# zahmedy/PyTorch-Distributed-Data-Parallel-DDP-Trainer

Measured on AMD Instinct MI355X. Metric: images/sec MNIST SimpleCNN DDP at 1/2/4/8 MI355X; DDP scaling efficiency, higher is better.
Workload: dtype bf16; 1 GPU; model=SimpleCNN (520,586 params), global_batch=32, per_rank_batch=32, image=1x28x28, parallelism=dp1, engine=fused hipGraph, graph_steps=7, graph_head=0, fuse_level=3, level3=True, params_finite=True, bucket_allreduce=none, params_identical_across_ranks=True, ranks_seen=1, force_allreduce=False, inlaunch_allreduce=False

## Files before the change

### csrc/bindings.cpp

```cpp
#include <torch/extension.h>
#include <c10/hip/HIPStream.h>

#include <optional>

#include "kernels/launchers.h"
#include "runtime/runtime.h"

namespace py = pybind11;
using at::Tensor;
using namespace ddp_amd;

extern "C" const char ddp_amd_source_hash_str[];

namespace {

hipStream_t cur_stream() { return c10::hip::getCurrentHIPStream().stream(); }

void check_cuda(const Tensor& t, const char* name) {
  TORCH_CHECK(t.is_cuda(), name, " must be a GPU tensor");
  TORCH_CHECK(t.is_contiguous(), name, " must be contiguous");
}
void check(const Tensor& t, const char* name, at::ScalarType st) {
  check_cuda(t, name);
  TORCH_CHECK(t.scalar_type() == st, name, " has dtype ", t.scalar_type(), ", expected ", st);
// ... 987 lines not shown
               b.a1 = bf(need("a1", at::kBFloat16, B * HW * c.C1));
               b.a2 = bf(need("a2", at::kBFloat16, B * HW * c.C2));
               b.dz2 = bf(need("dz2", at::kBFloat16, B * HW * c.C2));
               b.dz1 = bf(need("dz1", at::kBFloat16, B * HW * c.C1));
             }
             b.fc_part = need("fc_part", at::kFloat, 2L * conv3x3_dgrad_blocks(B, c.H, c.W, c.pxt_fwd) * c.NO).data_ptr<float>();
             b.dlogits = need("dlogits", at::kFloat, B * c.NO).data_ptr<float>();
             b.loss_rows = need("loss_rows", at::kFloat, B).data_ptr<float>();
             b.loss_hist = need("loss_hist", at::kFloat, 1).data_ptr<float>();
             b.w2slab = need("w2slab", at::kFloat, (long)conv3x3_wgrad_blocks(B, c.H, c.wgrad_rows) * (9L * c.C1 * c.C2 + c.C2)).data_ptr<float>();
             b.w1slab = need("w1slab", at::kFloat, (long)conv3x3_dgrad_blocks(B, c.H, c.W, c.pxt_dgrad) * 320).data_ptr<float>();
             b.step_ctr = need("step_ctr", at::kInt, 1).data_ptr<int>();
             b.xb = need("xb", at::kByte, B * HW).data_ptr<unsigned char>();
             b.yb = need("yb", at::kInt, B).data_ptr<int>();
             if (t.contains("sync_flags")) {
               long nfl = L3_IMG_OFF;
               if (c.fuse_level >= 3) nfl = std::max(nfl, (long)L3_IMG_OFF + (long)FWD_DZ_CNT_STRIDE * (B + 2));
               b.sync_flags = need("sync_flags", at::kInt, nfl).data_ptr<int>();
               b.sync_err = need("sync_err", at::kInt, 1).data_ptr<int>();
             }
             Tensor images = need("images", at::kByte, HW);
             b.images = images.data_ptr<unsigned char>();
             Tensor labels = need("labels", at::kInt, 1);
             b.labels = labels.data_ptr<int>();
             Tensor idx = need("idx", at::kInt, 1);
             b.idx = idx.data_ptr<int>();
             b.n_idx = (int)idx.numel();
             b.n_rows = (int)std::min<long>(images.numel() / HW, labels.numel());
             if (cfgd.contains("epoch_order") && cfgd["epoch_order"].cast<bool>()) b.idx = nullptr;
             TORCH_CHECK(conv3x3_wgrad_lds(c.W, c.C1, c.C2, c.wgrad_rows, true, es) <= 160 * 1024, "wgrad rows too large");
             return std::make_shared<SimpleCNNEngine>(c, b, comm, buckets);
           }),
// ... 26 lines not shown
```

### csrc/kernels/common.h

```cpp
#pragma once
#include <hip/hip_runtime.h>
#include <stdint.h>

#include "kernels/types.h"

namespace ddp_amd {

typedef __attribute__((ext_vector_type(8))) short bf16x8;
typedef __attribute__((ext_vector_type(4))) short bf16x4;
typedef __attribute__((ext_vector_type(4))) float f32x4;
typedef __attribute__((address_space(3))) bf16x4 lds_bf16x4;
typedef __attribute__((address_space(3))) char lds_char;
__device__ __forceinline__ lds_bf16x4* lds_ptr4(lds_char* base, int elem_off) {
  return (lds_bf16x4*)(base + 2 * elem_off);
}
typedef __attribute__((ext_vector_type(2))) __bf16 bf16x2v;

constexpr int WAVE = 64;

__device__ __forceinline__ void lds_barrier() {
  asm volatile("s_waitcnt lgkmcnt(0)\n\ts_barrier" ::: "memory");
}

namespace {
// ... 242 lines not shown
__device__ __forceinline__ float lane_bcast(float v, int lane) {
  return __builtin_bit_cast(float, __builtin_amdgcn_readlane(__builtin_bit_cast(int, v), lane));
}
__device__ __forceinline__ float wave_sum(float v) {
  v = row16_sum(v);
  return (lane_bcast(v, 0) + lane_bcast(v, 16)) + (lane_bcast(v, 32) + lane_bcast(v, 48));
}
__device__ __forceinline__ float sum16(float v) { return row16_sum(v); }
__device__ __forceinline__ float wave_max(float v) {
  v = row16_max(v);
  return fmaxf(fmaxf(lane_bcast(v, 0), lane_bcast(v, 16)), fmaxf(lane_bcast(v, 32), lane_bcast(v, 48)));
}

constexpr int XENT_MAX_BLK = 16;
constexpr int XENT_PRE_Q = 4;
template <typename Ld>
__device__ __forceinline__ float xent_logit_acc(int b, int o, int HW, int CH, int NO, Ld ld) {
  const int p0 = b * HW;
  const int kb0 = p0 / CH, kb1 = (p0 + HW - 1) / CH;
  const int slot0 = kb0 * CH == p0 ? 0 : 1;
  float a = 0.f;
#pragma unroll
  for (int j = 0; j < XENT_MAX_BLK; ++j) {
    const int kb = min(kb0 + j, kb1);
    const float v = ld((kb * 2 + (j == 0 ? slot0 : 0)) * NO + o);
    a += (kb0 + j <= kb1) ? v : 0.f;
  }
  return a;
}
__device__ __forceinline__ float xent_row_dl(const float* x, int NO, int o, int label, float gscale,
                                             float* loss) {
  label = label < 0 ? 0 : (label >= NO ? NO - 1 : label);
  float mx = x[0];
  for (int k = 1; k < NO; ++k) mx = fmaxf(mx, x[k]);
  float se = 0.f;
  for (int k = 0; k < NO; ++k) se += __expf(x[k] - mx);
  const float inv = 1.f / se;
  if (o == 0 && loss) *loss = mx + __logf(se) - x[label];
  return (__expf(x[o] - mx) * inv - (o == label ? 1.f : 0.f)) * gscale;
}
struct XentPre {
  int lab0;
  float bias_o;
// ... 78 lines not shown
```

### csrc/kernels/conv3x3.hip

```cpp
#include <algorithm>
#include <stdexcept>

#include <cstdio>
#include <cstdlib>

#include "kernels/conv3x3_fwd.h"

namespace ddp_amd {

size_t conv3x3_fwd_lds(int W, int Cin, int pxt, bool a1x, int es) {
  return fwd_stage_lds(W, Cin, pxt, a1x, es) + fc_epi_lds(pxt, FC_MAX_NOF);
}

size_t conv3x3_dgrad_lds(int W, int Cout, int pxt, bool fuse_w1, int es) {
  const size_t XR = 64 * pxt + 2 * W + 2;
  const int pad = es == 2 ? 16 : 8;
  return (size_t)es * ((size_t)32 * (9 * Cout + pad) + XR * (Cout + pad)) +
         (fuse_w1 ? sizeof(float) * (XR + 4 * 320) + 4 * 64 * pxt : 0);
}

bool conv3x3_fwd_dz_fits(int B, int H, int W, int pxt, int es) {
  return es == 4 ? fwd_dz_fits<float>(B, H, W, pxt) : fwd_dz_fits<bf16_t>(B, H, W, pxt);
}

// ... 29 lines not shown
bool conv3x3_step_head_fits(int nx, int B) {
  if (B <= 0 || nx <= 0) return false;
  const long nf = ((long)B * 28 * 28 + 63) / 64;
  const bool ok = (long)conv3x3_step_head_slots() >= nx + nf;
  if (!ok && std::getenv("DDP_AMD_XAR_DEBUG"))
    fprintf(stderr, "[ddp_amd] step head does not fit: %d resident slots < %ld blocks\n", conv3x3_step_head_slots(),
            nx + nf);
  return ok;
}

bool conv3x3_step_head(const BwdXar& x, int* done_fc, int* done_conv, const bf16_t* Wt, const float* bias,
                       bf16_t* Y, int B, const bf16_t* wfc, float* fc_part, const C1Src& c1, const FwdDz& dz,
                       int* err, hipStream_t s, const ShadowSet* late) {
  const int nx = x.nblk0 + x.nblk1;
  const char* bad = !x.args ? "all-reduce arguments" : x.nblk0 < 0 || x.nblk1 <= 0 ? "the conv bucket's blocks"
                   : !done_fc || !done_conv ? "bucket-done counters" : !dz.dz2 || !dz.img_cnt || !dz.fc_bias
                   ? "the level-3 forward's dZ2 outputs" : !wfc ? "the fc weight shadow" : !c1.x ? "the images" : nullptr;
  if (bad) throw std::runtime_error(std::string("conv3x3_step_head: missing ") + bad);
  if (!conv3x3_step_head_fits(nx, B)) return false;
  const long nf = ((long)B * 28 * 28 + 63) / 64;
  const size_t lds = std::max(conv3x3_fwd_lds(28, 32, 1, true, 2), (size_t)64 + sizeof(XgmiArgs));
  FwdMerge mg;
  mg.args = x.args;
  mg.nblk0 = x.nblk0;
  mg.nblk1 = x.nblk1;
  mg.fc_done = done_fc;
  mg.conv_done = done_conv;
  mg.err = err;
  if (late) mg.late = *late;
  auto k = step_head_kernel<bf16_t>;
  lds_optin(k, lds);
// ... 4 lines not shown
template <typename T>
static void fwd_launch(const T* X, const T* Wt, const float* bias, T* Y, int B, int H, int W, int Cin,
                       int Cout, bool relu, const T* wfc, float* fc_part, int pxt, hipStream_t s,
                       const C1Src* c1, const FwdDz* dz) {
  const long P = (long)B * H * W;
  const int per_blk = 64 * pxt;
  const dim3 grid((unsigned)((P + per_blk - 1) / per_blk), Cout / 64);
  const bool a1x = c1 != nullptr;
  const size_t lds = conv3x3_fwd_lds(W, Cin, pxt, a1x, (int)sizeof(T));
  const bool fc = wfc != nullptr;
  const C1Src cs = a1x ? *c1 : C1Src();
  const bool g = simplecnn_geom(H, W, Cin, Cout);
  const FwdDz dzo = dz ? *dz : FwdDz();
  if (dz) {
    if (!g || !fc || !a1x || !(pxt == 1 || pxt == 2) || !(sizeof(T) == 2 ? (void*)dz->dz2 : (void*)dz->dz2_f32) ||
        !dz->img_cnt || !dz->fc_bias)
      throw std::runtime_error("conv3x3_fwd: the level-3 dZ2 epilogue is the SimpleCNN forward with the fc "
                               "epilogue and the conv1 recompute");
    if constexpr (sizeof(T) == 2) {
      if (pxt == 2 && fwd_dz_occ2(grid.x)) {
        auto k = fwd_dz_kernel<T, 2, 2>();
        lds_optin(k, lds);
        hipLaunchKernelGGL(k, grid, dim3(512), lds, s, X, Wt, bias, Y, B, H, W, Cin, Cout, wfc, fc_part, cs, dzo);
        return;
      }
    }
    auto k = pxt == 2 ? fwd_dz_kernel<T, 2>() : fwd_dz_kernel<T, 1>();
    lds_optin(k, lds);
    hipLaunchKernelGGL(k, grid, dim3(256 * pxt), lds, s, X, Wt, bias, Y, B, H, W, Cin, Cout, wfc, fc_part, cs, dzo);
    return;
  }
// ... 143 lines not shown
```

### csrc/kernels/conv3x3_fwd.h

```cpp
#pragma once

#include "kernels/conv3x3_body.h"

namespace ddp_amd {

constexpr unsigned long long FWD_DZ_WAIT_TICKS = 2000000;
#ifndef DDP_AMD_F32_FC_PREFETCH
#define DDP_AMD_F32_FC_PREFETCH 0
#endif
constexpr bool F32_FC_PREFETCH = DDP_AMD_F32_FC_PREFETCH;
#ifndef DDP_AMD_FWD_PF_SPLIT
#define DDP_AMD_FWD_PF_SPLIT 1
#endif

struct FwdMerge {
  const XgmiArgs* args = nullptr;
  int nblk0 = 0, nblk1 = 0;
  int* fc_done = nullptr;
  int* conv_done = nullptr;
  int* err = nullptr;
  ShadowSet late{};
};
constexpr int MRG_ERR = 5;

// ... 117 lines not shown
```

### csrc/kernels/conv3x3_fwd_body.inc.h

```cpp
  using P = Prec<T>;
  constexpr bool F32 = sizeof(T) == 4;
  static_assert(!DZ || (NOF == 10 && A1X), "level-3 dZ2 needs the fc epilogue and the conv1 recompute");
  static_assert(!MRG || (DZ && !F32), "the merged forward is the bf16 level-3 forward");
  constexpr int CE = P::CE;
  DDP_STAMP(STAMP_K_CONV_FWD, 0);
  DDP_GEOM_OVERRIDE();
  constexpr int CH = 16 * NW * PXT, NT = NW * 64;
  const int lane = threadIdx.x & 63, wave = threadIdx.x >> 6;
  const int HW = H * W;
  const long Ptot = (long)B * HW;
  const int co0 = by * 64;
  const int KW = 9 * Cin, WS = KW + P::PAD, XS = Cin + P::PAD;
  const int XR = CH + 2 * W + 2;
  T* sW = reinterpret_cast<T*>(smem);
  T* sX = sW + 64 * WS;
  const long P0 = (long)bx * CH;
  const long Pbase = P0 - W - 1;

  const int wc = KW / CE;
  const int xc = Cin / CE;
  if (A1X && c1.zero_i32)
    for (int i = threadIdx.x; i < c1.zero_per_block; i += NT) {
      const long z = (long)bx * c1.zero_per_block + i;
      if (z < c1.zero_total) c1.zero_i32[z] = 0;
    }
  Conv1Group cg;
  if constexpr (!MRG) {
  if (A1X) cg = conv1_group_load(c1.w, c1.b, wave & 3);
  stage2<(64 / NW) * (F32 ? 2 : 1), NT>(64 * wc,
             [&](int i) { const int r = i / wc, c = (i - r * wc) * CE; return ld16(Wt + (long)(co0 + r) * KW + c); },
             [&](int i, bf16x8 v) { const int r = i / wc, c = (i - r * wc) * CE; st16(sW + r * WS + c, v); },
             A1X ? 0 : XR * xc,
             [&](int i) {
               const int r = i / xc, c = (i - r * xc) * CE;
               const long Pq = Pbase + r;
               return (Pq >= 0 && Pq < Ptot) ? ld16(X + Pq * Cin + c) : zero8();
             },
             [&](int i, bf16x8 v) { const int r = i / xc, c = (i - r * xc) * CE; st16(sX + r * XS + c, v); });
  }
  if (A1X) {
    float* sxx = reinterpret_cast<float*>(sX + XR * XS);
    const int NXX = XR + 2 * W + 2;
    const int base = c1.bi.base();
    for (int r = threadIdx.x; r < NXX; r += NT) {
      const long Pq = Pbase - W - 1 + r;
      float v = 0.f;
      if (Pq >= 0 && Pq < Ptot) {
        const int n = (int)(Pq / HW), rm = (int)(Pq - (long)n * HW);
        const int row = c1.bi.row(n, base);
        const unsigned char u = c1.x[(long)row * HW + rm];
        v = (float)u / 255.0f;
        if (c1.xb_out && Pq >= P0 && Pq < P0 + CH) {
          c1.xb_out[Pq] = u;
          if (rm == 0) c1.yb_out[n] = c1.labels[row];
        }
      }
      sxx[r] = v;
    }
// ... 217 lines not shown
    lds_barrier();
    if ((int)threadIdx.x < 2 * NOF) {
      const int slot = threadIdx.x / NOF, o = threadIdx.x - (threadIdx.x / NOF) * NOF;
      const long img = P0 / HW + slot;
      float acc_o = 0.f;
#pragma unroll
      for (int tile = 0; tile < NW * PXT; ++tile) {
        const long tp = P0 + tile * 16;
        const bool in = tp < Ptot && tp / HW == img;
#pragma unroll
        for (int g = 0; g < 4; ++g) {
          const float v = s_fc[(tile * 4 + g) * NOF + o];
          acc_o += in ? v : 0.f;
        }
      }
      float* dst = fc_part + ((long)bx * 2 + slot) * NOF + o;
      if constexpr (DZ || NOA2) st_wt(dst, acc_o);
      else *dst = acc_o;
    }
  }
  DDP_STAMP(STAMP_K_CONV_FWD, 4);
  if constexpr (DZ) {
    const int HWi = H * W;
    const int img0 = (int)(P0 / HWi);
    const long plast = (P0 + CH < Ptot ? P0 + CH : Ptot) - 1;
    const int nimg = (int)(plast / HWi) - img0 + 1;
    float* s_lg = s_fc + NW * PXT * 4 * NOF;
    float* s_dl = s_lg + 2 * NOF;
    auto store_a2 = [&]() {
#pragma unroll
      for (int pt = 0; pt < PXT; ++pt)
#pragma unroll
        for (int t = 0; t < 4; ++t) {
          const int co = co0 + 16 * t + 4 * (lane >> 4);
          if (!valid[pt]) continue;
          if constexpr (F32) st_wt(reinterpret_cast<float4*>(Y + Pp[pt] * Cout + co), a2q[pt][t]);
          else st_wt(reinterpret_cast<uint2*>(Y + Pp[pt] * Cout + co), a2pk[pt][t]);
        }
    };
    DDP_STAMP(STAMP_K_FWD_DZ, 0);
    if (wave != 0) store_a2();
    if (wave == 0) {
      int label = 0;
      if (lane < 2 * NOF) {
        const int im = img0 + (lane >= NOF ? 1 : 0);
        if (im < B) label = c1.labels[c1.bi.row(im, c1.bi.base())];
      }
      asm volatile("s_waitcnt vmcnt(0)" ::: "memory");
      DDP_STAMP(STAMP_K_FWD_DZ, 1);
      if (lane < nimg)
        __hip_atomic_fetch_add(dzo.img_cnt + (img0 + lane) * FWD_DZ_CNT_STRIDE, 1, __ATOMIC_RELAXED,
                               __HIP_MEMORY_SCOPE_AGENT);
      store_a2();
      {
        const int im = img0 + (lane < nimg ? lane : 0);
        const int kb0 = im * HWi / CH, kb1 = (im * HWi + HWi - 1) / CH;
        const int want = kb1 - kb0 + 1;
        const unsigned long long t0 = __builtin_amdgcn_s_memrealtime();
        while (true) {
          const int v = lane < nimg ? __hip_atomic_load(dzo.img_cnt + im * FWD_DZ_CNT_STRIDE, __ATOMIC_RELAXED,
                                                        __HIP_MEMORY_SCOPE_AGENT)
                                    : want;
          if (__all(v >= want)) break;
          if (__builtin_amdgcn_s_memrealtime() - t0 > FWD_DZ_WAIT_TICKS) {
            if (lane == 0 && dzo.err) __hip_atomic_store(dzo.err, 3, __ATOMIC_RELAXED, __HIP_MEMORY_SCOPE_AGENT);
            break;
          }
          __builtin_amdgcn_s_sleep(1);
        }
      }
      DDP_STAMP(STAMP_K_FWD_DZ, 2);
      if (lane < 2 * NOF) {
        const int slot = lane >= NOF ? 1 : 0, o = lane - slot * NOF;
        if (slot < nimg) {
          const float a = xent_logit_acc(img0 + slot, o, HWi, CH, NOF, [&](int i) {
            return __hip_atomic_load(fc_part + i, __ATOMIC_RELAXED, __HIP_MEMORY_SCOPE_AGENT);
          });
          s_lg[lane] = (MRG ? __hip_atomic_load(dzo.fc_bias + o, __ATOMIC_RELAXED, __HIP_MEMORY_SCOPE_AGENT)
                            : dzo.fc_bias[o]) + a;
        }
      }
      DDP_STAMP(STAMP_K_FWD_DZ, 4);
      asm volatile("s_waitcnt lgkmcnt(0)" ::: "memory");
      if (lane < 2 * NOF) {
        const int slot = lane >= NOF ? 1 : 0, o = lane - slot * NOF;
        if (slot < nimg) {
          float lossv = 0.f;
          const float d = xent_row_dl(s_lg + slot * NOF, NOF, o, label, dzo.gscale, &lossv);
          s_dl[lane] = d;
          if (dzo.dl_out && (slot == 1 || P0 == (long)img0 * HWi)) {
            const int im = img0 + slot;
            dzo.dl_out[im * NOF + o] = d;
            if (o == 0) dzo.loss_rows[im] = lossv;
          }
        }
      }
    }
    lds_barrier();
    DDP_STAMP(STAMP_K_FWD_DZ, 3);
#pragma unroll
    for (int pt = 0; pt < PXT; ++pt) {
      const long tp = P0 + (wave * PXT + pt) * 16;
      const float* dl = s_dl + (tp / HWi != img0 ? NOF : 0);
      float d[NOF];
#pragma unroll
      for (int o = 0; o < NOF; ++o) d[o] = dl[o];
#pragma unroll
      for (int t = 0; t < 4; ++t) {
        if constexpr (!PFW && !F32) __builtin_amdgcn_sched_barrier(0);
// ... 35 lines not shown
```

### csrc/kernels/fc_bwd_body.h

```cpp
#pragma once
#include "kernels/common.h"
#include "kernels/launchers.h"

namespace ddp_amd {

constexpr int FCB_RB = 8;

template <int CPL>
struct ColF {
  float v[CPL];
};
template <int CPL>
__device__ __forceinline__ ColF<CPL> ldc(const bf16_t* p) {
  ColF<CPL> r;
  if constexpr (CPL == 2) {
    const unsigned u = *reinterpret_cast<const unsigned*>(p);
    r.v[0] = __builtin_bit_cast(float, u << 16);
    r.v[1] = __builtin_bit_cast(float, u & 0xffff0000u);
  } else {
    const uint2 u = *reinterpret_cast<const uint2*>(p);
    r.v[0] = __builtin_bit_cast(float, u.x << 16);
    r.v[1] = __builtin_bit_cast(float, u.x & 0xffff0000u);
    r.v[2] = __builtin_bit_cast(float, u.y << 16);
    r.v[3] = __builtin_bit_cast(float, u.y & 0xffff0000u);
// ... 57 lines not shown
  if ((XENT || ex.loss_rows) && ex.loss_out) {
    const float* lr = XENT ? s_loss : ex.loss_rows;
    const int at = ex.step_ctr ? *ex.step_ctr : 0;
    float acc = 0.f;
    for (int b0 = 0; b0 < B; b0 += 64) {
      const float v = b0 + lane < B ? lr[b0 + lane] : 0.f;
      const int nb = B - b0 < 64 ? B - b0 : 64;
      for (int k = 0; k < nb; ++k)
        acc += __builtin_bit_cast(float, __builtin_amdgcn_readlane(__builtin_bit_cast(int, v), k));
    }
    if (lane == 63) {
      ex.loss_out[at] = acc / (float)B;
      if (last && ex.step_inc) *ex.step_inc = at + 1;
    }
  }
  if (ex.zero_i32 && (last || !ex.last_ctr))
    for (int i = lane; i < ex.n_zero; i += 64) ex.zero_i32[(long)i * ex.zero_stride] = 0;
}

constexpr int FCDW_LD = 12;
template <int MAXB, typename T>
__device__ __forceinline__ void fc_dw_wave_chunk(const float* s_dl, const T* __restrict__ X,
                                                 float* __restrict__ dW, float scale, int B, long K,
                                                 const FcBwdExtras& ex, long col0) {
  constexpr bool F32 = sizeof(T) == 4;
  constexpr int NO = 10, VW = 8, RPV = (MAXB + VW - 1) / VW;
  const int lane = threadIdx.x & 63;
  const long col = col0 + 2 * lane;
  const bool active = col < K;
  const long cc = active ? col : 0;
  typedef __attribute__((ext_vector_type(2))) int i32x2_t;
  const int vo4 = (int)cc * 4, vo2 = (int)cc * 2;
// ... 263 lines not shown
```

### csrc/kernels/launchers.h

```cpp
#pragma once
#include <hip/hip_runtime.h>
#include <stdint.h>

#include "kernels/types.h"

namespace ddp_amd {

void stamps_set(void* buf);

void conv1_fwd(const void* x, bool x_is_u8, BatchIdx bi, const float* w, const float* b, bf16_t* y,
               int B, int H, int W, int Cout, hipStream_t s);
void conv1_fwd(const void* x, bool x_is_u8, BatchIdx bi, const float* w, const float* b, float* y,
               int B, int H, int W, int Cout, hipStream_t s);
int conv1_wgrad_blocks(int B, int H, int W, int chunk);
void conv1_wgrad(const void* x, bool x_is_u8, BatchIdx bi, const bf16_t* dy, const bf16_t* yact,
                 float* slab, int B, int H, int W, int Cout, int chunk, hipStream_t s);
void conv1_wgrad(const void* x, bool x_is_u8, BatchIdx bi, const float* dy, const float* yact,
                 float* slab, int B, int H, int W, int Cout, int chunk, hipStream_t s);

constexpr int FWD_DZ_CNT_STRIDE = 64;
struct FwdDz {
  bf16_t* dz2 = nullptr;
  float* dz2_f32 = nullptr;
  int* img_cnt = nullptr;
  const float* fc_bias = nullptr;
  float gscale = 1.f;
  int* err = nullptr;
  float* dl_out = nullptr;
  float* loss_rows = nullptr;
};
bool conv3x3_fwd_dz_fits(int B, int H, int W, int pxt, int es = 2);
void conv3x3_fwd(const bf16_t* X, const bf16_t* Wt, const float* bias, bf16_t* Y, int B, int H,
                 int W, int Cin, int Cout, bool relu, const bf16_t* wfc, float* fc_part, int NO,
                 int pxt, hipStream_t s, const C1Src* c1 = nullptr, const FwdDz* dz = nullptr);
void conv3x3_fwd(const float* X, const float* Wt, const float* bias, float* Y, int B, int H,
                 int W, int Cin, int Cout, bool relu, const float* wfc, float* fc_part, int NO,
                 int pxt, hipStream_t s, const C1Src* c1 = nullptr, const FwdDz* dz = nullptr);
void conv3x3_dgrad(const bf16_t* dY, const bf16_t* Yact, const bf16_t* WT, const bf16_t* Xact,
                   bf16_t* dX, int B, int H, int W, int Cin, int Cout, const void* x0, bool x0_u8,
// ... 130 lines not shown
  const int* labels32 = nullptr;
  BatchIdx bi{};
  float gscale = 1.f;
  SgdArgs sgd{};
  float* p_w = nullptr;
  float* m_w = nullptr;
  bf16_t* sh_plain = nullptr;
  bf16_t* sh_frag = nullptr;
  float* sh_frag32 = nullptr;
  int frag_HW = 0, frag_C = 0;
  int sys_store = 0;
  int* last_ctr = nullptr;
  float* p_b = nullptr;
  float* m_b = nullptr;
  int* step_inc = nullptr;
  int* zero_i32 = nullptr;
  int n_zero = 0, zero_stride = 1;
  int last_n = 0;
};
struct BwdFc {
  const void* a2 = nullptr;
  const float* dl = nullptr;
  float* dW = nullptr;
  float scale = 1.f;
  long K = 0;
  int nconv = 0, fc0 = 0, nfc = 0;
  FcBwdExtras ex{};
};
size_t fc_bwd_lds(int B, int NO, bool xent, long npart = 0);
void noop(int blocks, int* sink, hipStream_t s);
// ... 109 lines not shown
```

### csrc/runtime/engine.cpp

```cpp
#include <algorithm>
#include <cstdio>
#include <cstdlib>
#include <cstring>

#include "runtime/runtime.h"

namespace ddp_amd {

SimpleCNNEngine::SimpleCNNEngine(const EngineConfig& cfg, const EngineBuffers& buf,
                                 std::shared_ptr<Comm> comm, std::vector<EngineBucket> buckets)
    : cfg_(cfg), b_(buf), comm_(std::move(comm)), buckets_(std::move(buckets)) {
  if (cfg_.C1 != 32) throw std::runtime_error("engine: fused conv1 wgrad needs C1 == 32");
  if (cfg_.C2 % 64 != 0) throw std::runtime_error("engine: C2 must be a multiple of 64");
  if ((cfg_.H * cfg_.W) % 16 != 0) throw std::runtime_error("engine: H*W must be a multiple of 16");
  if (cfg_.NO != 10) throw std::runtime_error("engine: the fused fc epilogue is built for 10 classes");
  if (cfg_.f32 && (cfg_.fuse_level < 1 || cfg_.store_a1 != 0))
    throw std::runtime_error("engine: fp32 mode needs fuse_level >= 1 (level 1 or 3) and store_a1 0");
  if (cfg_.f32 && !(b_.a2_f32 && b_.dz2_f32 && b_.w2t_f32 && b_.wfc_frag32))
    throw std::runtime_error("engine: fp32 mode needs the a2 / dz2 / w2t / wfc_frag32 fp32 buffers");
  const long conv0 = std::min(std::min(b_.off_w2, b_.off_b2), std::min(b_.off_w1, b_.off_b1));
  const long fc_hi = std::max(b_.off_wfc + (long)cfg_.NO * cfg_.H * cfg_.W * cfg_.C2, b_.off_bfc + cfg_.NO);
  if (fc_hi > conv0) throw std::runtime_error("engine: fc gradients must precede the conv gradients");
  long prev_end = 0;
  for (const EngineBucket& bk : buckets_) {
// ... 6 lines not shown
  for (int s : stage_) stage_used_[s] = true;
  xch_.assign(buckets_.size(), -1);
  DDP_HIP_CHECK(hipStreamCreateWithFlags(&cs_, hipStreamNonBlocking));
  DDP_HIP_CHECK(hipStreamCreateWithFlags(&ms_, hipStreamNonBlocking));
  for (hipEvent_t* e : {&e_b0_, &e_b1_, &e_d0_, &e_d1_, &e_fwd_, &e_fc_})
    DDP_HIP_CHECK(hipEventCreateWithFlags(e, hipEventDisableTiming));
  l3_fits_.assign(cfg_.max_batch + 1, -1);
  if (b_.sync_err) {
    DDP_HIP_CHECK(hipHostMalloc(reinterpret_cast<void**>(&err_host_), sizeof(int),
                                hipHostMallocCoherent | hipHostMallocMapped));
    *err_host_ = 0;
    int* dev = nullptr;
    DDP_HIP_CHECK(hipHostGetDevicePointer(reinterpret_cast<void**>(&dev), err_host_, 0));
    b_.sync_err = dev;
  }
}

SimpleCNNEngine::~SimpleCNNEngine() {
  if (process_exiting()) return;
  if (cs_) hipStreamSynchronize(cs_);
  destroy_graph();
  for (hipEvent_t e : {e_b0_, e_b1_, e_d0_, e_d1_, e_fwd_, e_fc_}) hipEventDestroy(e);
  for (XarArgs& e : xar_cache_) hipFree(const_cast<XgmiArgs*>(e.dev));
  if (err_host_) hipHostFree(err_host_);
}

void SimpleCNNEngine::destroy_graph() {
  if (graph_exec_) hipGraphExecDestroy(graph_exec_);
  if (graph_) hipGraphDestroy(graph_);
  graph_exec_ = nullptr;
  graph_ = nullptr;
  graph_steps_ = 0;
}

void SimpleCNNEngine::synchronize() {
  DDP_HIP_CHECK(hipStreamSynchronize(cs_));
  if (const int e = sync_error()) {
    throw std::runtime_error(std::string("engine: an in-launch hand-off wait timed out (") +
                             (e == 2 ? "fused slab reduction" : e == XAR_ERR ? "in-launch all-reduce"
// ... 79 lines not shown
  const bool pair_mode = dist && use_x && f1 && cfg_.dist_mode >= 3 && sync_ok_for_xar();
  if (fred || l3 || pair_mode) {
    const int nfwd = conv3x3_dgrad_blocks(B, H, W, cfg_.pxt_fwd);
    const int nsync = SYNC_RED_INTS + ((l3 || pair_mode) ? L3_FC_INTS : 0);
    c1.zero_i32 = b_.sync_flags;
    c1.zero_per_block = (nsync + nfwd - 1) / nfwd;
    c1.zero_total = nsync;
  }
  if (!l3 && plain_stale_) {
    refresh_shadows();
    plain_stale_ = false;
  }
  FwdDz dzo;
  if (l3) {
    dzo.dz2 = b_.dz2;
    dzo.img_cnt = b_.sync_flags + L3_IMG_OFF;
    dzo.fc_bias = P + b_.off_bfc;
    dzo.gscale = 1.f / (float)B;
    dzo.err = b_.sync_err;
    dzo.dl_out = b_.dlogits;
    dzo.loss_rows = b_.loss_rows;
  }
  const bool xar_mode = dist && use_x && l3 &&
                        ((cfg_.dist_mode == 2 && xar_plan_ok_) || cfg_.dist_mode >= 3);
  const bool one_stream = xar_mode || pair_mode;
  const bool fc_role = l3 && (!dist || xar_mode) && cfg_.l3_fc_role &&
                       conv3x3_bwd_fc_role_ok(H, W, C1, C2, cfg_.pxt_dgrad, cfg_.wgrad_split);
  const bool ov = dist && use_x && l3 && fc_role && cfg_.dist_mode == 4;
  if ((parts & (PART_HEAD | PART_AR)) && !ov && parts != PART_ALL)
    throw std::runtime_error("engine: a split step needs the dist_mode 4 chain");
  const C1Src* pc1 = f1 ? &c1 : nullptr;
// ... 14 lines not shown
  sh_all.count = l3 ? 3 : 4;
  const SgdArgs sa{cfg_.lr, cfg_.momentum, cfg_.dampening, cfg_.weight_decay, cfg_.nesterov,
                   cfg_.maximize, first_momentum_step ? 1 : 0, 1};
  float* M = b_.momentum;
  bool head_used = false;
  if (parts & PART_HEAD) {
    if (first_momentum_step) throw std::runtime_error("engine: the step head runs the steady-state SGD only");
    ShadowSet sh_head = sh_all, late{};
    if (late_shadow_ok(b_.off_w2, n_w2s)) {
      sh_head.r[1] = sh_all.r[2];
      sh_head.count = 2;
      late.r[0] = sh_all.r[1];
      late.count = 1;
    }
    BwdXar hx;
    int* mc = b_.sync_flags + L3_IMG_OFF + (long)FWD_DZ_CNT_STRIDE * cfg_.max_batch;
    if (cfg_.pxt_fwd == 1 && B == cfg_.max_batch) {
      if (!make_xar(hx, sa, M, sh_head)) throw std::runtime_error("engine: the step head needs the pair plan");
      hx.step_ctr = nullptr;
      head_used = conv3x3_step_head(hx, mc, mc + FWD_DZ_CNT_STRIDE, b_.w2_bf16, P + b_.off_b2, b_.a2, B,
                                    b_.wfc_frag, b_.fc_part, c1, dzo, b_.sync_err, cs_, &late);
    }
    if (!head_used) {
      if (!make_xar(hx, sa, M, sh_all)) throw std::runtime_error("engine: the step head needs the pair plan");
      hx.step_ctr = nullptr;
      xgmi_allreduce_pair(hx, cs_);
    }
    DDP_HIP_CHECK(hipGetLastError());
  }
  if ((parts & PART_FWD) || ((parts & PART_HEAD) && !head_used)) {
    if (!f1) conv1_fwd(b_.images, true, bi, P + b_.off_w1, P + b_.off_b1, b_.a1, B, H, W, C1, cs_);
// ... 27 lines not shown
  ex.sys_store = use_x ? 1 : 0;
  if (fopt) {
    ex.sgd = sa;
    ex.p_w = P + b_.off_wfc;
    ex.m_w = M ? M + b_.off_wfc : nullptr;
    ex.sh_plain = b_.wfc_bf16;
    ex.sh_frag = b_.wfc_frag;
    ex.frag_HW = HW;
    ex.frag_C = C2;
  }
  BwdFc fcr;
  std::function<void(hipStream_t)> fc_launch;
  if (l3) {
    ex.part = nullptr;
    ex.loss_rows = b_.loss_rows;
    ex.zero_i32 = dzo.img_cnt;
    ex.n_zero = ov ? cfg_.max_batch + 2 : B;
    ex.zero_stride = FWD_DZ_CNT_STRIDE;
    if (fc_role) {
      if (fopt) {
        ex.p_b = P + b_.off_bfc;
        ex.m_b = M ? M + b_.off_bfc : nullptr;
        ex.step_inc = b_.step_ctr;
      }
      if (ov) ex.step_inc = b_.step_ctr;
      ex.sh_plain = nullptr;
      fcr.a2 = b_.a2;
      fcr.dl = b_.dlogits;
      fcr.dW = fopt ? nullptr : G + b_.off_wfc;
      fcr.scale = inv_ws;
      fcr.K = (long)HW * C2;
      fcr.ex = ex;
    } else {
// ... 246 lines not shown
  const bool pair_mode = dist && use_x && cfg_.dist_mode >= 3 && sync_ok_for_xar();
  if (fred || l3 || pair_mode) {
    const int nfwd = conv3x3_dgrad_blocks(B, H, W, cfg_.pxt_fwd);
    const int nsync = SYNC_RED_INTS + ((l3 || pair_mode) ? L3_FC_INTS : 0);
    c1.zero_i32 = b_.sync_flags;
    c1.zero_per_block = (nsync + nfwd - 1) / nfwd;
    c1.zero_total = nsync;
  }
  const long n_w2 = (long)C2 * 9 * C1, w2row = n_w2 + C2, n_fc = (long)NO * HW * C2;
  const SgdArgs sa{cfg_.lr, cfg_.momentum, cfg_.dampening, cfg_.weight_decay, cfg_.nesterov,
                   cfg_.maximize, first_momentum_step ? 1 : 0, 1};
  const bool fopt = !dist && cfg_.fuse_opt;
  FwdDz dzo;
  if (l3) {
    dzo.dz2_f32 = b_.dz2_f32;
    dzo.img_cnt = b_.sync_flags + L3_IMG_OFF;
    dzo.fc_bias = P + b_.off_bfc;
    dzo.gscale = 1.f / (float)B;
    dzo.err = b_.sync_err;
    dzo.dl_out = b_.dlogits;
    dzo.loss_rows = b_.loss_rows;
  }
  const bool xar_mode = dist && use_x && l3 &&
                        ((cfg_.dist_mode == 2 && xar_plan_ok_) || cfg_.dist_mode >= 3);
  const bool one_stream = xar_mode || pair_mode;
  const bool fc_role = l3 && (!dist || xar_mode) && cfg_.l3_fc_role &&
                       conv3x3_bwd_fc_role_ok(H, W, C1, C2, cfg_.pxt_dgrad, cfg_.wgrad_split);

  conv3x3_fwd(static_cast<const float*>(nullptr), P + b_.off_w2, P + b_.off_b2, b_.a2_f32, B, H, W, C1, C2,
              true, b_.wfc_frag32, b_.fc_part, NO, cfg_.pxt_fwd, cs_, &c1, l3 ? &dzo : nullptr);
  FcBwdExtras ex;
  ex.dbias = G + b_.off_bfc;
  ex.dbias_scale = inv_ws;
  ex.loss_out = b_.loss_hist;
  ex.step_ctr = b_.step_ctr;
  ex.sys_store = use_x ? 1 : 0;
  if (l3) {
    ex.loss_rows = b_.loss_rows;
    ex.zero_i32 = dzo.img_cnt;
    ex.n_zero = B;
    ex.zero_stride = FWD_DZ_CNT_STRIDE;
  } else {
    ex.part = b_.fc_part;
    ex.HW = HW;
    ex.CH = 64 * cfg_.pxt_fwd;
    ex.fc_bias = P + b_.off_bfc;
    ex.labels32 = b_.yb;
    ex.bi = bid;
    ex.gscale = 1.f / (float)B;
  }
  if (fopt) {
    ex.sgd = sa;
    ex.p_w = P + b_.off_wfc;
    ex.m_w = M ? M + b_.off_wfc : nullptr;
    ex.sh_frag32 = b_.wfc_frag32;
    ex.frag_HW = HW;
// ... 176 lines not shown
```

### csrc/runtime/runtime.h

```cpp
#pragma once
#include <hip/hip_runtime.h>
#include <rccl/rccl.h>

#include <functional>
#include <memory>
#include <stdexcept>
#include <string>
#include <vector>

#include "kernels/launchers.h"
#include "runtime/bucket_state.h"

#define DDP_HIP_CHECK(expr)                                                              \
  do {                                                                                   \
    hipError_t _e = (expr);                                                              \
    if (_e != hipSuccess)                                                                \
      throw std::runtime_error(std::string("HIP error ") + hipGetErrorString(_e) + " at " + \
                               __FILE__ + ":" + std::to_string(__LINE__) + ": " #expr);  \
  } while (0)

#define DDP_NCCL_CHECK(expr)                                                             \
  do {                                                                                   \
    ncclResult_t _r = (expr);                                                            \
    if (_r != ncclSuccess)                                                               \
// ... 125 lines not shown
  float* wfc_frag32 = nullptr;
  bf16_t *a1, *a2, *dz2, *dz1;
  float *fc_part, *dlogits, *loss_rows, *loss_hist, *w2slab, *w1slab;
  int* step_ctr;
  unsigned char* xb;
  int* yb;
  int* sync_flags = nullptr;
  int* sync_err = nullptr;
  const unsigned char* images;
  const int* labels;
  const int* idx;
  int n_idx, n_rows;
};

constexpr int L3_FC_INTS = 32;
constexpr int L3_IMG_OFF = SYNC_RED_INTS + L3_FC_INTS;

struct EngineConfig {
  int max_batch, H, W, C1, C2, NO;
  int pxt_fwd, pxt_dgrad, wgrad_rows;
  int world, rank;
  float lr, momentum, dampening, weight_decay;
  int nesterov, maximize;
  int force_allreduce;
  int fuse_level = 0;
  int l3_fc_role = 1;
  int fuse_opt = 1;
  int store_a1 = 0;
  int f32 = 0;
  int fuse_reduce = 1;
  int wgrad_split = 1;
// ... 68 lines not shown
  bool last_xar_ = false;
  bool last_pair_ = false;
  bool last_head_ = false;
  bool capturing_ = false;
  int graph_heads_ = 0;
  bool xar_plan_ok_ = false;
  bool pair_plan_ok_ = false;
  struct XarArgs {
    XgmiArgs host[2];
    const XgmiArgs* dev = nullptr;
  };
  std::vector<XarArgs> xar_cache_;
  hipStream_t xs_ = nullptr;
  bool plain_stale_ = false;
  int* err_host_ = nullptr;
};

}
```

### pytorch-distributed-data-parallel-ddp-trainer_amd/engine/fused_step.py

```python
from __future__ import annotations

import dataclasses
import os
import math

import torch

from .. import native
from ..data.loader import DeviceMNIST
from ..data.sampler import ShardedSampler
from ..models.layers import flat_space
from ..ops.functional import wgrad_rows
from ..parallel.ddp import bucket_plan, bucket_ranges

from ..parallel.bucket_model import ONESHOT_MAX_ELEMS

BF16 = torch.bfloat16


@dataclasses.dataclass
class EngineOptions:
    graph_steps: int = 100
    use_graph: bool = True
    pxt_fwd: int | None = None
# ... 155 lines not shown
            **act,
            fc_part=e(2 * self.C.conv3x3_dgrad_blocks(B, 28, 28, self.opts.pxt_fwd) * 10),
            dlogits=e(B * 10), loss_rows=e(B),
            loss_hist=torch.zeros(self.steps_per_epoch + 1, device=dev),
            w2slab=e(self.C.conv3x3_wgrad_blocks(B, 28, R) * (64 * 9 * 32 + 64)),
            w1slab=e(self.C.conv3x3_dgrad_blocks(B, 28, 28, self.opts.pxt_dgrad) * 320),
            step_ctr=torch.zeros(1, dtype=torch.int32, device=dev),
            xb=torch.empty(B * HW, dtype=torch.uint8, device=dev),
            yb=torch.empty(B, dtype=torch.int32, device=dev),
            images=(torch.empty(n_rank * HW, dtype=torch.uint8, device=dev) if self.opts.epoch_order
                    else data.images_u8.view(-1)),
            labels=(torch.empty(n_rank, dtype=torch.int32, device=dev) if self.opts.epoch_order
                    else data.labels_i32),
            idx=torch.zeros(n_rank, dtype=torch.int32, device=dev),
        )
        nfl = 256 + 32 + 64 * (B + 2)
        self.t["sync_flags"] = torch.zeros(nfl, dtype=torch.int32, device=dev)
        self.t["sync_err"] = torch.zeros(1, dtype=torch.int32, device=dev)
        cfg = dict(max_batch=B, H=28, W=28, C1=32, C2=64, NO=10, pxt_fwd=self.opts.pxt_fwd,
                   pxt_dgrad=self.opts.pxt_dgrad, wgrad_rows=R, world=world_size, rank=rank,
                   lr=float(g["lr"]), momentum=float(g["momentum"]),
                   dampening=float(g["dampening"]), weight_decay=float(g["weight_decay"]),
                   nesterov=bool(g["nesterov"]), maximize=bool(g["maximize"]),
                   force_allreduce=bool(self.opts.force_allreduce),
                   fuse_level=self._fuse_level_ok(world_size), fuse_opt=bool(self.opts.fuse_opt),
                   store_a1=int(self.store_a1), f32=f32, fuse_reduce=self._fuse_reduce_ok(world_size),
                   epoch_order=bool(self.opts.epoch_order), wgrad_split=int(self.opts.wgrad_split),
                   l3_fc_role=int(self.opts.l3_fc_role), dist_mode=int(self.opts.dist_mode))
        self.dtype = "fp32" if f32 else "bf16"
        use_comm = world_size > 1 or self.opts.force_allreduce
        self.xgmi = None
# ... 439 lines not shown
```

Measured before the change: 960,600 images/sec.

## Replace per-image arrival counters with epoch-tagged fc partial slots in level-3 forward

The level-3 forward's fc epilogue now writes each partial logit together with a generation tag as a single 64-bit atomic store. The dZ wave polls those tagged slots directly instead of bumping and spinning on per-image counters and then re-reading the fc partials. This removes one atomic round trip, the per-image counter zeroing in the fc backward, and a separate load pass. In exchange it adds a separately allocated gran/gen buffer, a generation counter that the fc backward increments each step, and wider 64-bit polling loads split into sweeps.

```diff
diff --git a/csrc/bindings.cpp b/csrc/bindings.cpp
--- a/csrc/bindings.cpp
+++ b/csrc/bindings.cpp
@@ -1025,8 +1025,8 @@
              b.xb = need("xb", at::kByte, B * HW).data_ptr<unsigned char>();
              b.yb = need("yb", at::kInt, B).data_ptr<int>();
              if (t.contains("sync_flags")) {
-               long nfl = L3_IMG_OFF;
-               if (c.fuse_level >= 3) nfl = std::max(nfl, (long)L3_IMG_OFF + (long)FWD_DZ_CNT_STRIDE * (B + 2));
+               long nfl = L3_HEAD_OFF;
+               if (c.fuse_level >= 3) nfl = std::max(nfl, (long)L3_HEAD_OFF + (long)FWD_DZ_CNT_STRIDE * 2);
                b.sync_flags = need("sync_flags", at::kInt, nfl).data_ptr<int>();
                b.sync_err = need("sync_err", at::kInt, 1).data_ptr<int>();
              }
diff --git a/csrc/kernels/common.h b/csrc/kernels/common.h
--- a/csrc/kernels/common.h
+++ b/csrc/kernels/common.h
@@ -280,19 +280,27 @@
 
 constexpr int XENT_MAX_BLK = 16;
 constexpr int XENT_PRE_Q = 4;
-template <typename Ld>
-__device__ __forceinline__ float xent_logit_acc(int b, int o, int HW, int CH, int NO, Ld ld) {
+__device__ __forceinline__ int xent_logit_idx(int b, int o, int HW, int CH, int NO, int j) {
   const int p0 = b * HW;
   const int kb0 = p0 / CH, kb1 = (p0 + HW - 1) / CH;
   const int slot0 = kb0 * CH == p0 ? 0 : 1;
-  float a = 0.f;
-#pragma unroll
-  for (int j = 0; j < XENT_MAX_BLK; ++j) {
-    const int kb = min(kb0 + j, kb1);
-    const float v = ld((kb * 2 + (j == 0 ? slot0 : 0)) * NO + o);
+  const int kb = min(kb0 + j, kb1);
+  return (kb * 2 + (j == 0 ? slot0 : 0)) * NO + o;
+}
+template <int J0, int J1, typename Ld>
+__device__ __forceinline__ float xent_logit_acc_range(float a, int b, int o, int HW, int CH, int NO, Ld ld) {
+  const int p0 = b * HW;
+  const int kb0 = p0 / CH, kb1 = (p0 + HW - 1) / CH;
+#pragma unroll
+  for (int j = J0; j < J1; ++j) {
+    const float v = ld(j, xent_logit_idx(b, o, HW, CH, NO, j));
     a += (kb0 + j <= kb1) ? v : 0.f;
   }
   return a;
+}
+template <typename Ld>
+__device__ __forceinline__ float xent_logit_acc(int b, int o, int HW, int CH, int NO, Ld ld) {
+  return xent_logit_acc_range<0, XENT_MAX_BLK>(0.f, b, o, HW, CH, NO, [&](int, int i) { return ld(i); });
 }
 __device__ __forceinline__ float xent_row_dl(const float* x, int NO, int o, int label, float gscale,
                                              float* loss) {
diff --git a/csrc/kernels/conv3x3.hip b/csrc/kernels/conv3x3.hip
--- a/csrc/kernels/conv3x3.hip
+++ b/csrc/kernels/conv3x3.hip
@@ -67,7 +67,7 @@
                        int* err, hipStream_t s, const ShadowSet* late) {
   const int nx = x.nblk0 + x.nblk1;
   const char* bad = !x.args ? "all-reduce arguments" : x.nblk0 < 0 || x.nblk1 <= 0 ? "the conv bucket's blocks"
-                   : !done_fc || !done_conv ? "bucket-done counters" : !dz.dz2 || !dz.img_cnt || !dz.fc_bias
+                   : !done_fc || !done_conv ? "bucket-done counters" : !dz.dz2 || !dz.gran || !dz.gen || !dz.fc_bias
                    ? "the level-3 forward's dZ2 outputs" : !wfc ? "the fc weight shadow" : !c1.x ? "the images" : nullptr;
   if (bad) throw std::runtime_error(std::string("conv3x3_step_head: missing ") + bad);
   if (!conv3x3_step_head_fits(nx, B)) return false;
@@ -102,7 +102,7 @@
   const FwdDz dzo = dz ? *dz : FwdDz();
   if (dz) {
     if (!g || !fc || !a1x || !(pxt == 1 || pxt == 2) || !(sizeof(T) == 2 ? (void*)dz->dz2 : (void*)dz->dz2_f32) ||
-        !dz->img_cnt || !dz->fc_bias)
+        !dz->gran || !dz->gen || !dz->fc_bias)
       throw std::runtime_error("conv3x3_fwd: the level-3 dZ2 epilogue is the SimpleCNN forward with the fc "
                                "epilogue and the conv1 recompute");
     if constexpr (sizeof(T) == 2) {
diff --git a/csrc/kernels/conv3x3_fwd.h b/csrc/kernels/conv3x3_fwd.h
--- a/csrc/kernels/conv3x3_fwd.h
+++ b/csrc/kernels/conv3x3_fwd.h
@@ -1,4 +1,6 @@
 #pragma once
+
+#include <type_traits>
 
 #include "kernels/conv3x3_body.h"
 
diff --git a/csrc/kernels/conv3x3_fwd_body.inc.h b/csrc/kernels/conv3x3_fwd_body.inc.h
--- a/csrc/kernels/conv3x3_fwd_body.inc.h
+++ b/csrc/kernels/conv3x3_fwd_body.inc.h
@@ -5,6 +5,13 @@
   constexpr int CE = P::CE;
   DDP_STAMP(STAMP_K_CONV_FWD, 0);
   DDP_GEOM_OVERRIDE();
+  typedef __attribute__((address_space(1))) unsigned long long gran_t;
+  constexpr int DZ_SW = (OCC == 2 || F32) ? XENT_MAX_BLK / 2 : XENT_MAX_BLK;
+  unsigned dz_epoch = 1u;
+  if constexpr (DZ) {
+    const unsigned g = *dzo.gen + 1u;
+    dz_epoch = g ? g : 1u;
+  }
   constexpr int CH = 16 * NW * PXT, NT = NW * 64;
   const int lane = threadIdx.x & 63, wave = threadIdx.x >> 6;
   const int HW = H * W;
@@ -25,6 +32,7 @@
       if (z < c1.zero_total) c1.zero_i32[z] = 0;
     }
   Conv1Group cg;
+  int bi_base = 0;
   if constexpr (!MRG) {
   if (A1X) cg = conv1_group_load(c1.w, c1.b, wave & 3);
   stage2<(64 / NW) * (F32 ? 2 : 1), NT>(64 * wc,
@@ -41,7 +49,7 @@
   if (A1X) {
     float* sxx = reinterpret_cast<float*>(sX + XR * XS);
     const int NXX = XR + 2 * W + 2;
-    const int base = c1.bi.base();
+    const int base = bi_base = c1.bi.base();
     for (int r = threadIdx.x; r < NXX; r += NT) {
       const long Pq = Pbase - W - 1 + r;
       float v = 0.f;
@@ -289,9 +297,15 @@
           acc_o += in ? v : 0.f;
         }
       }
-      float* dst = fc_part + ((long)bx * 2 + slot) * NOF + o;
-      if constexpr (DZ || NOA2) st_wt(dst, acc_o);
-      else *dst = acc_o;
+      if constexpr (DZ) {
+        __hip_atomic_store((gran_t*)dzo.gran + ((long)bx * 2 + slot) * NOF + o,
+                           ((unsigned long long)dz_epoch << 32) | __builtin_bit_cast(unsigned, acc_o),
+                           __ATOMIC_RELAXED, __HIP_MEMORY_SCOPE_AGENT);
+      } else {
+        float* dst = fc_part + ((long)bx * 2 + slot) * NOF + o;
+        if constexpr (NOA2) st_wt(dst, acc_o);
+        else *dst = acc_o;
+      }
     }
   }
   DDP_STAMP(STAMP_K_CONV_FWD, 4);
@@ -314,60 +328,66 @@
         }
     };
     DDP_STAMP(STAMP_K_FWD_DZ, 0);
-    if (wave != 0) store_a2();
+    store_a2();
     if (wave == 0) {
+      const int slot = lane >= NOF ? 1 : 0, o = lane - slot * NOF;
+      const bool act = lane < 2 * NOF && slot < nimg;
       int label = 0;
+      float fcb = 0.f;
       if (lane < 2 * NOF) {
-        const int im = img0 + (lane >= NOF ? 1 : 0);
-        if (im < B) label = c1.labels[c1.bi.row(im, c1.bi.base())];
-      }
-      asm volatile("s_waitcnt vmcnt(0)" ::: "memory");
+        const int im = img0 + slot;
+        if (im < B) label = c1.labels[c1.bi.row(im, bi_base)];
+        fcb = MRG ? __hip_atomic_load(dzo.fc_bias + o, __ATOMIC_RELAXED, __HIP_MEMORY_SCOPE_AGENT) : dzo.fc_bias[o];
+      }
+      const int im = img0 + (act ? slot : 0);
+      const int nblk = (im * HWi + HWi - 1) / CH - im * HWi / CH + 1;
+      const gran_t* gr = (const gran_t*)dzo.gran;
+      const unsigned long long t0 = __builtin_amdgcn_s_memrealtime();
+      bool dead = false;
+      float a = 0.f;
       DDP_STAMP(STAMP_K_FWD_DZ, 1);
-      if (lane < nimg)
-        __hip_atomic_fetch_add(dzo.img_cnt + (img0 + lane) * FWD_DZ_CNT_STRIDE, 1, __ATOMIC_RELAXED,
-                               __HIP_MEMORY_SCOPE_AGENT);
-      store_a2();
-      {
-        const int im = img0 + (lane < nimg ? lane : 0);
-        const int kb0 = im * HWi / CH, kb1 = (im * HWi + HWi - 1) / CH;
-        const int want = kb1 - kb0 + 1;
-        const unsigned long long t0 = __builtin_amdgcn_s_memrealtime();
-        while (true) {
-          const int v = lane < nimg ? __hip_atomic_load(dzo.img_cnt + im * FWD_DZ_CNT_STRIDE, __ATOMIC_RELAXED,
-                                                        __HIP_MEMORY_SCOPE_AGENT)
-                                    : want;
-          if (__all(v >= want)) break;
+      auto sweep = [&](auto j0c) {
+        constexpr int J0 = decltype(j0c)::value;
+        unsigned long long g[DZ_SW];
+#pragma unroll
+        for (int k = 0; k < DZ_SW; ++k) g[k] = 0;
+        const bool none = J0 > 0 && !__any(act && nblk > J0);
+        while (!none) {
+          bool ok = true;
+          if (act) {
+#pragma unroll
+            for (int k = 0; k < DZ_SW; ++k)
+              g[k] = __hip_atomic_load(gr + xent_logit_idx(im, o, HWi, CH, NOF, J0 + k), __ATOMIC_RELAXED,
+                                       __HIP_MEMORY_SCOPE_AGENT);
+#pragma unroll
+            for (int k = 0; k < DZ_SW; ++k) ok &= (unsigned)(g[k] >> 32) == dz_epoch;
+          }
+          if (__all(ok) || dead) break;
           if (__builtin_amdgcn_s_memrealtime() - t0 > FWD_DZ_WAIT_TICKS) {
             if (lane == 0 && dzo.err) __hip_atomic_store(dzo.err, 3, __ATOMIC_RELAXED, __HIP_MEMORY_SCOPE_AGENT);
+            dead = true;
             break;
           }
           __builtin_amdgcn_s_sleep(1);
         }
-      }
+        a = xent_logit_acc_range<J0, J0 + DZ_SW>(a, im, o, HWi, CH, NOF, [&](int j, int) {
+          return __builtin_bit_cast(float, (unsigned)g[j - J0]);
+        });
+      };
+      sweep(std::integral_constant<int, 0>{});
+      if constexpr (DZ_SW < XENT_MAX_BLK) sweep(std::integral_constant<int, DZ_SW>{});
       DDP_STAMP(STAMP_K_FWD_DZ, 2);
-      if (lane < 2 * NOF) {
-        const int slot = lane >= NOF ? 1 : 0, o = lane - slot * NOF;
-        if (slot < nimg) {
-          const float a = xent_logit_acc(img0 + slot, o, HWi, CH, NOF, [&](int i) {
-            return __hip_atomic_load(fc_part + i, __ATOMIC_RELAXED, __HIP_MEMORY_SCOPE_AGENT);
-          });
-          s_lg[lane] = (MRG ? __hip_atomic_load(dzo.fc_bias + o, __ATOMIC_RELAXED, __HIP_MEMORY_SCOPE_AGENT)
-                            : dzo.fc_bias[o]) + a;
-        }
-      }
+      asm volatile("" : "+v"(label));
+      if (act) s_lg[lane] = fcb + a;
       DDP_STAMP(STAMP_K_FWD_DZ, 4);
       asm volatile("s_waitcnt lgkmcnt(0)" ::: "memory");
-      if (lane < 2 * NOF) {
-        const int slot = lane >= NOF ? 1 : 0, o = lane - slot * NOF;
-        if (slot < nimg) {
-          float lossv = 0.f;
-          const float d = xent_row_dl(s_lg + slot * NOF, NOF, o, label, dzo.gscale, &lossv);
-          s_dl[lane] = d;
-          if (dzo.dl_out && (slot == 1 || P0 == (long)img0 * HWi)) {
-            const int im = img0 + slot;
-            dzo.dl_out[im * NOF + o] = d;
-            if (o == 0) dzo.loss_rows[im] = lossv;
-          }
+      if (act) {
+        float lossv = 0.f;
+        const float d = xent_row_dl(s_lg + slot * NOF, NOF, o, label, dzo.gscale, &lossv);
+        s_dl[lane] = d;
+        if (dzo.dl_out && (slot == 1 || P0 == (long)img0 * HWi)) {
+          dzo.dl_out[im * NOF + o] = d;
+          if (o == 0) dzo.loss_rows[im] = lossv;
         }
       }
     }
diff --git a/csrc/kernels/fc_bwd_body.h b/csrc/kernels/fc_bwd_body.h
--- a/csrc/kernels/fc_bwd_body.h
+++ b/csrc/kernels/fc_bwd_body.h
@@ -95,8 +95,14 @@
       if (last && ex.step_inc) *ex.step_inc = at + 1;
     }
   }
-  if (ex.zero_i32 && (last || !ex.last_ctr))
-    for (int i = lane; i < ex.n_zero; i += 64) ex.zero_i32[(long)i * ex.zero_stride] = 0;
+  if (last || !ex.last_ctr) {
+    if (ex.zero_i32)
+      for (int i = lane; i < ex.n_zero; i += 64) ex.zero_i32[(long)i * ex.zero_stride] = 0;
+    if (ex.gen_inc && lane == 0) {
+      const unsigned g = *ex.gen_inc + 1u;
+      *ex.gen_inc = g == 0xffffffffu ? 0u : g;
+    }
+  }
 }
 
 constexpr int FCDW_LD = 12;
diff --git a/csrc/kernels/launchers.h b/csrc/kernels/launchers.h
--- a/csrc/kernels/launchers.h
+++ b/csrc/kernels/launchers.h
@@ -22,7 +22,8 @@
 struct FwdDz {
   bf16_t* dz2 = nullptr;
   float* dz2_f32 = nullptr;
-  int* img_cnt = nullptr;
+  unsigned long long* gran = nullptr;
+  const unsigned* gen = nullptr;
   const float* fc_bias = nullptr;
   float gscale = 1.f;
   int* err = nullptr;
@@ -183,6 +184,7 @@
   float* p_b = nullptr;
   float* m_b = nullptr;
   int* step_inc = nullptr;
+  unsigned* gen_inc = nullptr;
   int* zero_i32 = nullptr;
   int n_zero = 0, zero_stride = 1;
   int last_n = 0;
diff --git a/csrc/runtime/engine.cpp b/csrc/runtime/engine.cpp
--- a/csrc/runtime/engine.cpp
+++ b/csrc/runtime/engine.cpp
@@ -44,6 +44,14 @@
     DDP_HIP_CHECK(hipHostGetDevicePointer(reinterpret_cast<void**>(&dev), err_host_, 0));
     b_.sync_err = dev;
   }
+  if (cfg_.fuse_level >= 3 && b_.sync_flags && b_.sync_err) {
+    const size_t ng = 2 * (size_t)cfg_.NO * (size_t)conv3x3_dgrad_blocks(cfg_.max_batch, cfg_.H, cfg_.W, 1);
+    DDP_HIP_CHECK(hipMalloc(reinterpret_cast<void**>(&gran_), ng * sizeof(unsigned long long)));
+    DDP_HIP_CHECK(hipMalloc(reinterpret_cast<void**>(&gen_), 256));
+    DDP_HIP_CHECK(hipMemset(gran_, 0, ng * sizeof(unsigned long long)));
+    DDP_HIP_CHECK(hipMemset(gen_, 0, 256));
+    DDP_HIP_CHECK(hipStreamSynchronize(nullptr));
+  }
 }
 
 SimpleCNNEngine::~SimpleCNNEngine() {
@@ -53,6 +61,8 @@
   for (hipEvent_t e : {e_b0_, e_b1_, e_d0_, e_d1_, e_fwd_, e_fc_}) hipEventDestroy(e);
   for (XarArgs& e : xar_cache_) hipFree(const_cast<XgmiArgs*>(e.dev));
   if (err_host_) hipHostFree(err_host_);
+  if (gran_) hipFree(gran_);
+  if (gen_) hipFree(gen_);
 }
 
 void SimpleCNNEngine::destroy_graph() {
@@ -162,7 +172,8 @@
   FwdDz dzo;
   if (l3) {
     dzo.dz2 = b_.dz2;
-    dzo.img_cnt = b_.sync_flags + L3_IMG_OFF;
+    dzo.gran = gran_;
+    dzo.gen = gen_;
     dzo.fc_bias = P + b_.off_bfc;
     dzo.gscale = 1.f / (float)B;
     dzo.err = b_.sync_err;
@@ -207,7 +218,7 @@
       late.count = 1;
     }
     BwdXar hx;
-    int* mc = b_.sync_flags + L3_IMG_OFF + (long)FWD_DZ_CNT_STRIDE * cfg_.max_batch;
+    int* mc = b_.sync_flags + L3_HEAD_OFF;
     if (cfg_.pxt_fwd == 1 && B == cfg_.max_batch) {
       if (!make_xar(hx, sa, M, sh_head)) throw std::runtime_error("engine: the step head needs the pair plan");
       hx.step_ctr = nullptr;
@@ -265,9 +276,12 @@
   if (l3) {
     ex.part = nullptr;
     ex.loss_rows = b_.loss_rows;
-    ex.zero_i32 = dzo.img_cnt;
-    ex.n_zero = ov ? cfg_.max_batch + 2 : B;
-    ex.zero_stride = FWD_DZ_CNT_STRIDE;
+    ex.gen_inc = gen_;
+    if (ov) {
+      ex.zero_i32 = b_.sync_flags + L3_HEAD_OFF;
+      ex.n_zero = 2;
+      ex.zero_stride = FWD_DZ_CNT_STRIDE;
+    }
     if (fc_role) {
       if (fopt) {
         ex.p_b = P + b_.off_bfc;
@@ -544,7 +558,8 @@
   FwdDz dzo;
   if (l3) {
     dzo.dz2_f32 = b_.dz2_f32;
-    dzo.img_cnt = b_.sync_flags + L3_IMG_OFF;
+    dzo.gran = gran_;
+    dzo.gen = gen_;
     dzo.fc_bias = P + b_.off_bfc;
     dzo.gscale = 1.f / (float)B;
     dzo.err = b_.sync_err;
@@ -567,9 +582,7 @@
   ex.sys_store = use_x ? 1 : 0;
   if (l3) {
     ex.loss_rows = b_.loss_rows;
-    ex.zero_i32 = dzo.img_cnt;
-    ex.n_zero = B;
-    ex.zero_stride = FWD_DZ_CNT_STRIDE;
+    ex.gen_inc = gen_;
   } else {
     ex.part = b_.fc_part;
     ex.HW = HW;
diff --git a/csrc/runtime/runtime.h b/csrc/runtime/runtime.h
--- a/csrc/runtime/runtime.h
+++ b/csrc/runtime/runtime.h
@@ -163,7 +163,7 @@
 };
 
 constexpr int L3_FC_INTS = 32;
-constexpr int L3_IMG_OFF = SYNC_RED_INTS + L3_FC_INTS;
+constexpr int L3_HEAD_OFF = SYNC_RED_INTS + L3_FC_INTS;
 
 struct EngineConfig {
   int max_batch, H, W, C1, C2, NO;
@@ -262,6 +262,8 @@
   hipStream_t xs_ = nullptr;
   bool plain_stale_ = false;
   int* err_host_ = nullptr;
+  unsigned long long* gran_ = nullptr;
+  unsigned* gen_ = nullptr;
 };
 
 }
diff --git a/pytorch-distributed-data-parallel-ddp-trainer_amd/engine/fused_step.py b/pytorch-distributed-data-parallel-ddp-trainer_amd/engine/fused_step.py
--- a/pytorch-distributed-data-parallel-ddp-trainer_amd/engine/fused_step.py
+++ b/pytorch-distributed-data-parallel-ddp-trainer_amd/engine/fused_step.py
@@ -193,7 +193,7 @@
                     else data.labels_i32),
             idx=torch.zeros(n_rank, dtype=torch.int32, device=dev),
         )
-        nfl = 256 + 32 + 64 * (B + 2)
+        nfl = 256 + 32 + 64 * 2
         self.t["sync_flags"] = torch.zeros(nfl, dtype=torch.int32, device=dev)
         self.t["sync_err"] = torch.zeros(1, dtype=torch.int32, device=dev)
         cfg = dict(max_batch=B, H=28, W=28, C1=32, C2=64, NO=10, pxt_fwd=self.opts.pxt_fwd,
```

Measured after the change: 1.007 million images/sec (median of 6 runs). 1.05x the previous value.
